# nktoan/h-edit

Measured on AMD Instinct MI355X. Metric: edited images/sec (512^2, 50 steps, K Langevin), higher is better.
Workload: dtype bf16

## Files before the change

### h-edit_amd/csrc/c_api.hip

```cpp
#include "../../include/hedit.h"
#include <exception>
#include <map>
#include <mutex>
#include <new>
#include <set>
#include <utility>

#include "common.h"
#include "kernels.h"

static thread_local std::string g_last_error;
void hedit_set_error(const std::string& msg) { g_last_error = msg; }

int hedit_abi_catch() noexcept {
  try {
    try {
      throw;
    } catch (const std::bad_alloc&) {
      g_last_error = "out of host memory inside libhedit_hip";
    } catch (const std::exception& e) {
      g_last_error = std::string("C++ exception inside libhedit_hip: ") + e.what();
    } catch (...) {
      g_last_error = "unknown C++ exception inside libhedit_hip";
    }
// ... 133 lines not shown
int hedit_k_gemm_plan_splits(int M, int N, int K, int chunk_kt) { return gemm_plan_splits(M, N, K, chunk_kt); }

int hedit_k_gemm(const void* A, const void* W, const float* bias, const void* residual, void* C, int M, int N,
                 int K, int lda, int ldc, int ldr, int mode, int Hin, int Win, int Cin, int Hout, int Wout,
                 int splits, void* partial_ws, void* stream) try {
  ARG_CHECK(A && W && C, "gemm args");
  GemmParams p{};
  p.A = reinterpret_cast<const bf16_t*>(A);
  p.W = reinterpret_cast<const bf16_t*>(W);
  p.M = M; p.N = N; p.K = K; p.lda = lda; p.mode = mode;
  p.Hin = Hin; p.Win = Win; p.Cin = Cin; p.Hout = Hout; p.Wout = Wout;
  p.bias = bias;
  p.residual = reinterpret_cast<const bf16_t*>(residual);
  p.ldr = ldr;
  p.C = reinterpret_cast<bf16_t*>(C);
  p.ldc = ldc;
  if (splits < 0) {
    const int kt = K / 64;
    const int s = gemm_pick_splits(M, N, K, -splits);
    p.chunk_kt = (kt + s - 1) / s;
    return gemm_launch(p, 1, nullptr, S(stream));
  }
  const int s = gemm_pick_splits(M, N, K, splits);
  return gemm_launch(p, s, reinterpret_cast<float*>(partial_ws), S(stream));
} catch (...) { return hedit_abi_catch(); }

int hedit_k_conv_gn(const void* A, const void* W, const float* bias, const void* residual, void* C, int M, int N, int K, int ldc,
                    int ldr, int mode, int Hin, int Win, int Cin, int Hout, int Wout, int splits, void* partial_ws, float* gn_part,
                    void* stream) try {
  ARG_CHECK(A && W && C && gn_part, "conv_gn args");
  GemmParams p{};
  p.A = reinterpret_cast<const bf16_t*>(A);
  p.W = reinterpret_cast<const bf16_t*>(W);
  p.M = M; p.N = N; p.K = K; p.lda = Cin; p.mode = mode;
  p.Hin = Hin; p.Win = Win; p.Cin = Cin; p.Hout = Hout; p.Wout = Wout;
  p.bias = bias;
  p.residual = reinterpret_cast<const bf16_t*>(residual);
  p.ldr = ldr;
  p.C = reinterpret_cast<bf16_t*>(C);
  p.ldc = ldc;
  p.gn_part = gn_part;
  if (splits < 0) {
    const int kt = K / 64;
    const int s = gemm_pick_splits(M, N, K, -splits);
    p.chunk_kt = (kt + s - 1) / s;
    return gemm_launch(p, 1, nullptr, S(stream));
  }
  const int s = gemm_pick_splits(M, N, K, splits);
  return gemm_launch(p, s, reinterpret_cast<float*>(partial_ws), S(stream));
} catch (...) { return hedit_abi_catch(); }

int hedit_k_groupnorm_from_parts(const void* x, void* y, const float* gamma, const float* beta, int B, int HW, int C, int G,
                                 float eps, int silu, const float* part_a, int ca, const float* part_b, int cb, void* ws,
                                 void* stream) try {
  ARG_CHECK(x && y && gamma && beta && part_a && ws, "groupnorm_from_parts args");
  return groupnorm_from_parts_launch(reinterpret_cast<const bf16_t*>(x), reinterpret_cast<bf16_t*>(y), gamma, beta, B, HW, C, G,
                                     eps, silu, part_a, ca, part_b, cb, reinterpret_cast<float*>(ws), S(stream));
} catch (...) { return hedit_abi_catch(); }

int hedit_k_pack_geglu(const float* w, const float* bias, void* w_packed_bf16, float* bias_packed, int inner, int K,
                       void* stream) try {
  ARG_CHECK(w && w_packed_bf16, "pack_geglu args");
  int rc = pack_geglu_rows_launch(w, reinterpret_cast<bf16_t*>(w_packed_bf16), nullptr, 2 * inner, K, S(stream));
  if (rc != HEDIT_OK || !bias) return rc;
  ARG_CHECK(bias_packed, "pack_geglu: bias_packed");
  return pack_geglu_rows_launch(bias, nullptr, bias_packed, 2 * inner, 1, S(stream));
} catch (...) { return hedit_abi_catch(); }

int hedit_k_gemm_geglu(const void* A, const void* w_packed, const float* bias_packed, void* C, int M, int inner, int K,
                       int lda, int ldc, void* stream) try {
  ARG_CHECK(A && w_packed && C, "gemm_geglu args");
  GemmParams p{};
  p.A = reinterpret_cast<const bf16_t*>(A);
  p.W = reinterpret_cast<const bf16_t*>(w_packed);
  p.M = M; p.N = 2 * inner; p.K = K; p.lda = lda; p.mode = 0;
  p.bias = bias_packed;
  p.C = reinterpret_cast<bf16_t*>(C);
  p.ldc = ldc;
  p.geglu = 1;
  return gemm_launch(p, 1, nullptr, S(stream));
} catch (...) { return hedit_abi_catch(); }

int hedit_k_ffn_channels(void) { return ffn_fused_channels(); }
size_t hedit_k_ffn_stream_bytes(int with_outer_layers) { return ffn_stream_bytes(with_outer_layers, with_outer_layers); }
size_t hedit_k_ffn_bias_bytes(void) { return ffn_bias_bytes(); }

int hedit_k_ffn_pack(const float* w1, const float* b1, const float* w2, const float* w_pre, const float* w_post, void* stream_out,
                     float* bias1_out, void* stream) try {
  ARG_CHECK(w1 && b1 && w2 && stream_out && bias1_out && ((w_pre == nullptr) == (w_post == nullptr)), "ffn_pack args");
  const int outer = w_pre != nullptr;
  bf16_t* so = reinterpret_cast<bf16_t*>(stream_out);
  int rc = ffn_pack_launch(w1, 1, outer, outer, so, S(stream));
  if (rc == HEDIT_OK) rc = ffn_pack_launch(w2, 2, outer, outer, so, S(stream));
  if (rc == HEDIT_OK && outer) rc = ffn_pack_launch(w_pre, 0, 1, 1, so, S(stream));
  if (rc == HEDIT_OK && outer) rc = ffn_pack_launch(w_post, 3, 1, 1, so, S(stream));
  if (rc != HEDIT_OK) return rc;
  return ffn_pack_bias_launch(b1, bias1_out, S(stream));
} catch (...) { return hedit_abi_catch(); }

int hedit_k_ffn_fused(const void* x, int64_t ldx, const float* gamma, const float* beta, float eps, const void* w_stream,
                      const float* bias1_packed, const float* bias2, void* out, int64_t ldo, int M, int C, void* stream) try {
  FfnParams f{};
  f.x = reinterpret_cast<const bf16_t*>(x); f.ldx = (long)ldx; f.gamma = gamma; f.beta = beta; f.eps = eps;
  f.stream = reinterpret_cast<const bf16_t*>(w_stream); f.bias1p = bias1_packed; f.bias2 = bias2;
  f.out = reinterpret_cast<bf16_t*>(out); f.ldo = (long)ldo; f.M = M; f.C = C;
  return ffn_fused_launch(f, S(stream));
} catch (...) { return hedit_abi_catch(); }

int hedit_k_ffn_chain(const void* a, int64_t lda, const void* t1, int64_t ldt1, const void* x, int64_t ldx, const float* bias_pre,
                      const float* gamma, const float* beta, float eps, const void* w_stream, const float* bias1_packed, const float* bias2,
                      const float* bias_post, void* out, int64_t ldo, int M, int C, void* stream) try {
  ARG_CHECK(a && t1 && x, "ffn_chain args");
  FfnParams f{};
  f.a = reinterpret_cast<const bf16_t*>(a); f.lda = (long)lda;
  f.x = reinterpret_cast<const bf16_t*>(t1); f.ldx = (long)ldt1;
  f.r2 = reinterpret_cast<const bf16_t*>(x); f.ldr2 = (long)ldx;
  f.bias_pre = bias_pre; f.bias_post = bias_post;
  f.gamma = gamma; f.beta = beta; f.eps = eps;
  f.stream = reinterpret_cast<const bf16_t*>(w_stream); f.bias1p = bias1_packed; f.bias2 = bias2;
  f.out = reinterpret_cast<bf16_t*>(out); f.ldo = (long)ldo; f.M = M; f.C = C;
  return ffn_fused_launch(f, S(stream));
} catch (...) { return hedit_abi_catch(); }

size_t hedit_k_lin_chain_stream_bytes(int n_out) { return lin_chain_stream_bytes(n_out == 3 ? 4 : 2); }

int hedit_k_lin_chain_pack(const float* w_pre, const float* w0, const float* w1, const float* w2, float scale0, void* stream_out,
                           void* stream) try {
  ARG_CHECK(w_pre && w0 && stream_out && ((w1 == nullptr) == (w2 == nullptr)), "lin_chain_pack args");
  const int layers = w1 ? 4 : 2;
  bf16_t* so = reinterpret_cast<bf16_t*>(stream_out);
  int rc = lin_chain_pack_launch(w_pre, 0, 1.f, layers, so, S(stream));
  if (rc == HEDIT_OK) rc = lin_chain_pack_launch(w0, 1, scale0, layers, so, S(stream));
  if (rc == HEDIT_OK && w1) rc = lin_chain_pack_launch(w1, 2, 1.f, layers, so, S(stream));
  if (rc == HEDIT_OK && w1) rc = lin_chain_pack_launch(w2, 3, 1.f, layers, so, S(stream));
  return rc;
} catch (...) { return hedit_abi_catch(); }

int hedit_k_lin_chain(const void* a, int64_t lda, const void* r1, int64_t ldr1, const float* gn_ss, int rows_per_image,
                      const float* bias_pre, const float* gamma, const float* beta, float eps, const void* w_stream, void* out_mid,
                      int64_t ldmid, void* out_q, int64_t ldq, void* out_k, int64_t ldk, void* out, int64_t ldo, int M, int C,
                      void* stream) try {
  LinChainParams c{};
  c.a = reinterpret_cast<const bf16_t*>(a); c.lda = (long)lda; c.r1 = reinterpret_cast<const bf16_t*>(r1); c.ldr1 = (long)ldr1;
  c.bias_pre = bias_pre; c.gamma = gamma; c.beta = beta; c.eps = eps; c.stream = reinterpret_cast<const bf16_t*>(w_stream);
  c.out_mid = reinterpret_cast<bf16_t*>(out_mid); c.ldmid = (long)ldmid; c.out = reinterpret_cast<bf16_t*>(out); c.ldo = (long)ldo;
  c.M = M; c.C = C; c.gn_ss = gn_ss; c.rows_per_image = rows_per_image;
  c.out_q = reinterpret_cast<bf16_t*>(out_q); c.ldq = (long)ldq; c.out_k = reinterpret_cast<bf16_t*>(out_k); c.ldk = (long)ldk;
  return lin_chain_launch(c, S(stream));
} catch (...) { return hedit_abi_catch(); }

int hedit_storage_is_f16(void) { return HEDIT_F16; }

int hedit_test_set_flags(int flags) try {
  ARG_CHECK(flags >= 0 && flags <= 15, "hedit_test_set_flags: bit 0 drained ring waits, bit 1 exact self-attention pass, bit 2 pixel-UNet GroupNorm statistics path flipped, bit 3 no persistent linear kernel");
  g_test_flags.store(flags, std::memory_order_relaxed);
  return HEDIT_OK;
} catch (...) { return hedit_abi_catch(); }

int hedit_k_lin_chain_sched(const void* a, int64_t lda, const void* r1, int64_t ldr1, const float* gn_ss, int rows_per_image,
                            const float* bias_pre, const float* gamma, const float* beta, float eps, const void* w_stream, void* out_mid,
                            int64_t ldmid, void* out_q, int64_t ldq, void* out_k, int64_t ldk, void* out, int64_t ldo, int M, int C,
                            int sched, void* stream) try {
  LinChainParams c{};
  c.a = reinterpret_cast<const bf16_t*>(a); c.lda = (long)lda; c.r1 = reinterpret_cast<const bf16_t*>(r1); c.ldr1 = (long)ldr1;
  c.bias_pre = bias_pre; c.gamma = gamma; c.beta = beta; c.eps = eps; c.stream = reinterpret_cast<const bf16_t*>(w_stream);
  c.out_mid = reinterpret_cast<bf16_t*>(out_mid); c.ldmid = (long)ldmid; c.out = reinterpret_cast<bf16_t*>(out); c.ldo = (long)ldo;
  c.M = M; c.C = C; c.gn_ss = gn_ss; c.rows_per_image = rows_per_image;
  c.out_q = reinterpret_cast<bf16_t*>(out_q); c.ldq = (long)ldq; c.out_k = reinterpret_cast<bf16_t*>(out_k); c.ldk = (long)ldk;
  return lin_chain_launch_sched(c, sched, S(stream));
} catch (...) { return hedit_abi_catch(); }

size_t hedit_k_groupnorm_ws_bytes(int B, int HW, int C) { return groupnorm_ws_bytes(B, HW, C); }

int hedit_k_groupnorm_affine(const void* x, const float* gamma, const float* beta, int B, int HW, int C, int G, float eps, void* ws,
                             float* ss_out, void* stream) try {
  ARG_CHECK(x && gamma && beta && ws && ss_out, "groupnorm_affine args");
  const float* ss = nullptr;
  int rc = groupnorm_affine_launch(reinterpret_cast<const bf16_t*>(x), gamma, beta, B, HW, C, G, eps, reinterpret_cast<float*>(ws), S(stream), &ss);
  if (rc != HEDIT_OK) return rc;
  HIP_TRY(hipMemcpyAsync(ss_out, ss, (size_t)B * C * 2 * sizeof(float), hipMemcpyDeviceToDevice, S(stream)));
  return HEDIT_OK;
} catch (...) { return hedit_abi_catch(); }

int hedit_k_groupnorm(const void* x, void* y, const float* gamma, const float* beta, int B, int HW, int C, int G,
                      float eps, int silu, void* ws, void* stream) try {
  ARG_CHECK(x && y && gamma && beta && ws, "groupnorm args");
  return groupnorm_launch(reinterpret_cast<const bf16_t*>(x), reinterpret_cast<bf16_t*>(y), gamma, beta, B, HW, C, G,
                          eps, silu, reinterpret_cast<float*>(ws), S(stream));
} catch (...) { return hedit_abi_catch(); }

int hedit_k_layernorm(const void* x, void* y, const float* gamma, const float* beta, int64_t rows, int C, float eps,
                      void* stream) try {
  ARG_CHECK(x && y && gamma && beta, "layernorm args");
  return layernorm_launch(reinterpret_cast<const bf16_t*>(x), reinterpret_cast<bf16_t*>(y), gamma, beta, (long)rows, C, eps, S(stream));
} catch (...) { return hedit_abi_catch(); }

int hedit_k_geglu(const void* x, void* y, int64_t rows, int inner, void* stream) try {
  ARG_CHECK(x && y, "geglu args");
  return geglu_launch(reinterpret_cast<const bf16_t*>(x), reinterpret_cast<bf16_t*>(y), (long)rows, inner, S(stream));
} catch (...) { return hedit_abi_catch(); }

int hedit_k_self_attn(const void* q, int ldq, const void* k, int ldk, const void* vt, int64_t ldvt, void* out, int ldo,
                      int B, int N, int heads, int d, const int32_t* qk_src, const int32_t* kv_src, void* stream) try {
  ARG_CHECK(q && k && vt && out, "self_attn args");
  SelfAttnParams p{};
  p.q = reinterpret_cast<const bf16_t*>(q); p.ldq = ldq;
  p.k = reinterpret_cast<const bf16_t*>(k); p.ldk = ldk;
  p.vt = reinterpret_cast<const bf16_t*>(vt); p.ldvt = (long)ldvt;
  p.out = reinterpret_cast<bf16_t*>(out); p.ldo = ldo;
  p.B = B; p.N = N; p.heads = heads; p.d = d; p.qk_src = qk_src; p.kv_src = kv_src;
  return self_attn_launch(p, S(stream));
} catch (...) { return hedit_abi_catch(); }

int hedit_k_cross_attn(const void* q, int ldq, const void* k, int ldk, const void* vt, int64_t ldvt, void* out, int ldo,
                       int B, int N, int heads, int d, const hedit_p2p_plan* plan, float* store, void* stream) try {
  ARG_CHECK(q && k && vt && out && plan, "cross_attn args");
  CrossAttnParams p{};
  p.q = reinterpret_cast<const bf16_t*>(q); p.ldq = ldq;
  p.k = reinterpret_cast<const bf16_t*>(k); p.ldk = ldk;
  p.vt = reinterpret_cast<const bf16_t*>(vt); p.ldvt = (long)ldvt;
  p.out = reinterpret_cast<bf16_t*>(out); p.ldo = ldo;
  p.B = B; p.N = N; p.heads = heads; p.d = d;
  p.n_pairs = plan->n_pairs; p.pair_src = plan->pair_src; p.pair_tar = plan->pair_tar;
  p.mixT = reinterpret_cast<const bf16_t*>(plan->mixT); p.bvec = plan->bvec;
  p.singles = plan->singles; p.n_single = plan->n_single;
  p.store = store;
  return cross_attn_launch(p, S(stream));
} catch (...) { return hedit_abi_catch(); }

int hedit_k_attn_probs(const void* q, int ldq, const void* k, int ldk, float* probs, int B, int N, int M, int kstride,
                       int heads, int d, void* stream) try {
  ARG_CHECK(q && k && probs, "attn_probs args");
  AttnProbsParams p{};
  p.q = reinterpret_cast<const bf16_t*>(q); p.ldq = ldq;
  p.k = reinterpret_cast<const bf16_t*>(k); p.ldk = ldk;
  p.probs = probs; p.B = B; p.N = N; p.M = M; p.kstride = kstride; p.heads = heads; p.d = d;
  return attn_probs_launch(p, S(stream));
} catch (...) { return hedit_abi_catch(); }

int hedit_k_attn_apply(const float* probs, const void* vt, int64_t ldvt, void* out, int ldo, int B, int N, int M,
                       int kstride, int heads, int d, void* stream) try {
  ARG_CHECK(probs && vt && out, "attn_apply args");
  AttnProbsParams p{};
  p.probs = const_cast<float*>(probs);
  p.vt = reinterpret_cast<const bf16_t*>(vt); p.ldvt = (long)ldvt;
  p.out = reinterpret_cast<bf16_t*>(out); p.ldo = ldo;
  p.B = B; p.N = N; p.M = M; p.kstride = kstride; p.heads = heads; p.d = d;
  return attn_apply_launch(p, S(stream));
} catch (...) { return hedit_abi_catch(); }

int hedit_k_pack_conv3x3(const float* w, void* out, int O, int I, void* stream) try {
  ARG_CHECK(w && out, "pack args");
  return pack_conv3x3_launch(w, reinterpret_cast<bf16_t*>(out), O, I, S(stream));
} catch (...) { return hedit_abi_catch(); }

int hedit_k_f32_to_bf16(const float* x, void* y, int64_t n, void* stream) try {
  ARG_CHECK(x && y, "cast args");
  return f32_to_bf16_launch(x, reinterpret_cast<bf16_t*>(y), (long)n, S(stream));
} catch (...) { return hedit_abi_catch(); }

int hedit_k_groupnorm_stats(const void* x, void* y, const float* gamma, const float* beta, int B, int HW, int C, int G,
                            float eps, int silu, void* ws, float* stats, void* stream) try {
  ARG_CHECK(x && y && gamma && beta && ws && stats, "groupnorm_stats args");
  return groupnorm_launch(reinterpret_cast<const bf16_t*>(x), reinterpret_cast<bf16_t*>(y), gamma, beta, B, HW, C, G,
                          eps, silu, reinterpret_cast<float*>(ws), S(stream), stats);
} catch (...) { return hedit_abi_catch(); }

size_t hedit_k_groupnorm_bwd_ws_bytes(int B, int HW, int C) { return groupnorm_bwd_ws_bytes(B, HW, C); }

int hedit_k_groupnorm_bwd(const void* x, const void* dy, const void* add, void* dx, const float* gamma, const float* beta,
                          const float* stats, int B, int HW, int C, int G, int silu, void* ws, void* stream) try {
  ARG_CHECK(x && dy && dx && gamma && beta && stats && ws, "groupnorm_bwd args");
  return groupnorm_bwd_launch(reinterpret_cast<const bf16_t*>(x), reinterpret_cast<const bf16_t*>(dy),
                              reinterpret_cast<const bf16_t*>(add), reinterpret_cast<bf16_t*>(dx), gamma, beta, stats, B, HW, C,
                              G, silu, reinterpret_cast<float*>(ws), S(stream));
} catch (...) { return hedit_abi_catch(); }

int hedit_k_softmax_rows(const float* s, void* p, int64_t rows, int N, float scale, void* stream) try {
  ARG_CHECK(s && p, "softmax_rows args");
  return softmax_rows_launch(s, reinterpret_cast<bf16_t*>(p), (long)rows, N, scale, S(stream));
} catch (...) { return hedit_abi_catch(); }

int hedit_k_softmax_blockdiag(const float* s, void* p, int64_t rows, int T, int ld, float scale, void* stream) try {
  ARG_CHECK(s && p, "softmax_blockdiag args");
  return softmax_blockdiag_launch(s, reinterpret_cast<bf16_t*>(p), (long)rows, T, ld, scale, S(stream));
} catch (...) { return hedit_abi_catch(); }

int hedit_k_softmax_bwd(const void* p, const float* dp, void* ds, int64_t rows, int N, float scale, void* stream) try {
  ARG_CHECK(p && dp && ds, "softmax_bwd args");
  return softmax_bwd_launch(reinterpret_cast<const bf16_t*>(p), dp, reinterpret_cast<bf16_t*>(ds), (long)rows, N, scale, S(stream));
} catch (...) { return hedit_abi_catch(); }

int hedit_k_transpose(const void* src, void* dst, int R, int C, void* stream) try {
  ARG_CHECK(src && dst, "transpose args");
  return transpose_bf16_launch(reinterpret_cast<const bf16_t*>(src), reinterpret_cast<bf16_t*>(dst), R, C, S(stream));
} catch (...) { return hedit_abi_catch(); }

int hedit_k_sum2x2(const void* du, void* dx, int B, int H, int W, int C, void* stream) try {
  ARG_CHECK(du && dx, "sum2x2 args");
  return sum2x2_launch(reinterpret_cast<const bf16_t*>(du), reinterpret_cast<bf16_t*>(dx), B, H, W, C, S(stream));
} catch (...) { return hedit_abi_catch(); }

int hedit_k_pack_conv3x3_dgrad(const float* w, void* out, int O, int I, void* stream) try {
  ARG_CHECK(w && out, "pack args");
  return pack_conv3x3_dgrad_launch(w, reinterpret_cast<bf16_t*>(out), O, I, S(stream));
} catch (...) { return hedit_abi_catch(); }

// ... 110 lines not shown
```

### h-edit_amd/csrc/norm.hip

```cpp
#include <stdlib.h>
#include "common.h"
#include "kernels.h"

namespace {


constexpr int GN_MAXV = 2;

__global__ __launch_bounds__(256) void gn_partial_kernel(const bf16_t* __restrict__ x, float* __restrict__ part,
                                                         int HW, int C, int G, int nslab) {
  extern __shared__ float lds[];
  const int CV = C / 8;
  const int slab = blockIdx.x, b = blockIdx.y;
  const int pix_per = (HW + nslab - 1) / nslab;
  const int p0 = slab * pix_per;
  int p1 = p0 + pix_per;
  if (p1 > HW) p1 = HW;
  const int R = CV <= 256 ? 256 / CV : 1;
  const int r = CV <= 256 ? threadIdx.x / CV : 0;
  const int cv0 = CV <= 256 ? threadIdx.x % CV : threadIdx.x;
  const bool active = r < R;
  float s[GN_MAXV][8], q[GN_MAXV][8];
#pragma unroll
  for (int v = 0; v < GN_MAXV; ++v)
// ... 450 lines not shown
  }
  acc = wave_sum(acc);
  if (lane == 0) out[n] = acc + (b0 ? b0[n] : 0.f) + (b1 ? b1[n] : 0.f);
}

__global__ void timestep_embed_kernel(float t, float* out, int dim) {
  const int half = dim / 2;
  for (int i = threadIdx.x; i < half; i += blockDim.x) {
    const float fr = expf(-9.210340371976184f * (float)i / (float)half);
    const float a = t * fr;
    out[i] = cosf(a);
    out[half + i] = sinf(a);
  }
}

__global__ void timestep_embed_ddpm_kernel(float t, float* out, int dim) {
  const int half = dim / 2;
  for (int i = threadIdx.x; i < half; i += blockDim.x) {
    const float fr = expf(-9.210340371976184f / (float)(half - 1) * (float)i);
    const float a = t * fr;
    out[i] = sinf(a);
    out[half + i] = cosf(a);
  }
  if ((dim & 1) && threadIdx.x == 0) out[dim - 1] = 0.f;
}

constexpr int CI_PIX = 128;
__global__ __launch_bounds__(256) void conv_in_kernel(const float* __restrict__ x, const float* __restrict__ w, const float* __restrict__ bias,
                                                      bf16_t* __restrict__ y, int B, int Cin, int H, int Wd, int Cout) {
  extern __shared__ float lds[];
  const int K = Cin * 9;
  float* sw = lds;
  float* sx = lds + (long)K * Cout;
  for (int i = threadIdx.x; i < K * Cout; i += 256) {
    const int co = i / K, k = i - co * K;
    sw[k * Cout + co] = w[i];
  }
  const long pix0 = (long)blockIdx.x * CI_PIX;
  const long npix = (long)B * H * Wd;
  for (int i = threadIdx.x; i < CI_PIX * K; i += 256) {
    const int k = i / CI_PIX, pl = i - k * CI_PIX;
    const long pix = pix0 + pl;
    float v = 0.f;
    if (pix < npix) {
      const int ox = (int)(pix % Wd), oy = (int)((pix / Wd) % H), b = (int)(pix / ((long)Wd * H));
      const int ci = k / 9, tap = k - ci * 9;
      const int iy = oy + tap / 3 - 1, ix = ox + tap % 3 - 1;
      if ((unsigned)iy < (unsigned)H && (unsigned)ix < (unsigned)Wd) v = x[(((long)b * Cin + ci) * H + iy) * Wd + ix];
    }
    sx[k * CI_PIX + pl] = v;
  }
  __syncthreads();
  const int CV = Cout / 8;
  for (int i = threadIdx.x; i < (CI_PIX / 4) * CV; i += 256) {
    const int pg = i / CV, cv = i - pg * CV;
    float acc[4][8];
#pragma unroll
    for (int q = 0; q < 4; ++q)
#pragma unroll
      for (int j = 0; j < 8; ++j) acc[q][j] = bias[cv * 8 + j];
    for (int k = 0; k < K; ++k) {
      const float4 xv = *reinterpret_cast<const float4*>(sx + k * CI_PIX + pg * 4);
      const float4 w0 = *reinterpret_cast<const float4*>(sw + k * Cout + cv * 8);
      const float4 w1 = *reinterpret_cast<const float4*>(sw + k * Cout + cv * 8 + 4);
      const float xq[4] = {xv.x, xv.y, xv.z, xv.w};
#pragma unroll
      for (int q = 0; q < 4; ++q) {
        acc[q][0] += xq[q] * w0.x; acc[q][1] += xq[q] * w0.y; acc[q][2] += xq[q] * w0.z; acc[q][3] += xq[q] * w0.w;
        acc[q][4] += xq[q] * w1.x; acc[q][5] += xq[q] * w1.y; acc[q][6] += xq[q] * w1.z; acc[q][7] += xq[q] * w1.w;
      }
    }
#pragma unroll
    for (int q = 0; q < 4; ++q) {
      const long pix = pix0 + pg * 4 + q;
      if (pix < npix) *reinterpret_cast<uint4*>(y + pix * Cout + cv * 8) = pack8(acc[q]);
    }
  }
}

__global__ __launch_bounds__(256) void conv_out_kernel(const bf16_t* __restrict__ x, const bf16_t* __restrict__ w, const float* __restrict__ bias,
                                                       float* __restrict__ y, int B, int H, int Wd, int C, int Cout) {
  const int lane = threadIdx.x & 63;
  const long pix = (long)blockIdx.x * 4 + (threadIdx.x >> 6);
  if (pix >= (long)B * H * Wd) return;
  const int ox = (int)(pix % Wd);
  const int oy = (int)((pix / Wd) % H);
  const int b = (int)(pix / ((long)Wd * H));
  const int CV = C / 8;
  float acc[4] = {0.f, 0.f, 0.f, 0.f};
  for (int idx = lane; idx < 9 * CV; idx += 64) {
    const int tap = idx / CV, cv = idx - tap * CV;
    const int iy = oy + tap / 3 - 1, ix = ox + tap % 3 - 1;
    if ((unsigned)iy >= (unsigned)H || (unsigned)ix >= (unsigned)Wd) continue;
    uint4 u = *reinterpret_cast<const uint4*>(x + (((long)b * H + iy) * Wd + ix) * C + cv * 8);
    float f[8];
    unpack8(u, f);
    for (int co = 0; co < Cout; ++co) {
      uint4 uw = *reinterpret_cast<const uint4*>(w + ((long)co * 9 + tap) * C + cv * 8);
      float ww[8];
      unpack8(uw, ww);
#pragma unroll
      for (int j = 0; j < 8; ++j) acc[co] += f[j] * ww[j];
    }
  }
  for (int co = 0; co < Cout; ++co) {
    float v = wave_sum(acc[co]);
    if (lane == 0) y[(((long)b * Cout + co) * H + oy) * Wd + ox] = v + bias[co];
  }
}

__global__ __launch_bounds__(256) void gn_small_kernel(const bf16_t* __restrict__ x, bf16_t* __restrict__ y,
                                                       const float* __restrict__ gamma, const float* __restrict__ beta,
                                                       int HW, int C, int G, float eps, int silu, float* __restrict__ stats) {
  extern __shared__ uint32_t gs_pairs[];
  __shared__ float red[8];
  const int g = blockIdx.x, b = blockIdx.y, tid = threadIdx.x;
  const int cpg = C / G, ppp = cpg / 2;
  const int npair = HW * ppp;
  const uint32_t* xin = reinterpret_cast<const uint32_t*>(x + (long)b * HW * C + g * cpg);
  float s = 0.f, q = 0.f;
  for (int i = tid; i < npair; i += 256) {
    const int pix = i / ppp, j = i - pix * ppp;
    const uint32_t u = xin[(long)pix * (C / 2) + j];
    gs_pairs[i] = u;
    const float a = st_lo(u), c = st_hi(u);
    s += a; s += c;
    q += a * a; q += c * c;
  }
  s = wave_sum(s);
  q = wave_sum(q);
  if ((tid & 63) == 0) { red[(tid >> 6) * 2] = s; red[(tid >> 6) * 2 + 1] = q; }
  __syncthreads();
  s = ((red[0] + red[2]) + red[4]) + red[6];
  q = ((red[1] + red[3]) + red[5]) + red[7];
  const float n = (float)HW * (float)cpg;
  const float m = s / n;
  float var = q / n - m * m;
  var = var < 0.f ? 0.f : var;
  const float rstd = rsqrtf(var + eps);
  if (stats && tid == 0) *reinterpret_cast<float2*>(stats + ((long)b * G + g) * 2) = make_float2(m, rstd);
  uint32_t* yout = reinterpret_cast<uint32_t*>(y + (long)b * HW * C + g * cpg);
  for (int i = tid; i < npair; i += 256) {
    const int pix = i / ppp, j = i - pix * ppp;
    const uint32_t u = gs_pairs[i];
    const int c0 = g * cpg + 2 * j;
    const float sc0 = rstd * gamma[c0], sc1 = rstd * gamma[c0 + 1];
    float a = st_lo(u) * sc0 + (beta[c0] - m * sc0);
    float c = st_hi(u) * sc1 + (beta[c0 + 1] - m * sc1);
    if (silu) { a = silu_f(a); c = silu_f(c); }
    yout[(long)pix * (C / 2) + j] = pack_bf16x2(a, c);
  }
}

__global__ __launch_bounds__(256) void gn_fold_kernel(const float* __restrict__ pa, int npa, const float* __restrict__ pb, int npb,
                                                      float* __restrict__ out, int units, int ppg) {
  __shared__ float red[8];
  const int g = blockIdx.x, b = blockIdx.y, tid = threadIdx.x;
  const int total = units * ppg;
  float s = 0.f, q = 0.f;
  for (int e = tid; e < total; e += 256) {
    const int u = e / ppg, j = e - u * ppg;
    const int pr = g * ppg + j;
    const long row = (long)b * units + u;
    const float2 v = pr < npa ? *reinterpret_cast<const float2*>(pa + (row * npa + pr) * 2)
                              : *reinterpret_cast<const float2*>(pb + (row * npb + (pr - npa)) * 2);
    s += v.x;
    q += v.y;
  }
  s = wave_sum(s);
  q = wave_sum(q);
  if ((tid & 63) == 0) { red[(tid >> 6) * 2] = s; red[(tid >> 6) * 2 + 1] = q; }
  __syncthreads();
  if (tid == 0) {
    s = ((red[0] + red[2]) + red[4]) + red[6];
    q = ((red[1] + red[3]) + red[5]) + red[7];
    *reinterpret_cast<float2*>(out + ((long)b * gridDim.x + g) * 2) = make_float2(s, q);
  }
}

int gn_nslab(int B, int HW, int C) {
  (void)B;
  const int CV = C / 8;
  const int R = CV <= 256 ? 256 / CV : 1;
  int n = HW / (R * 8);
  int cap = HW / 256;
  cap = cap < 32 ? 32 : (cap > 64 ? 64 : cap);
  if (HW >= 512 * 512) cap = 128;
  if (n > cap) n = cap;
  if (n < 1) n = 1;
  return n;
}

}

size_t groupnorm_ws_bytes(int B, int HW, int C) {
  const int nslab = gn_nslab(B, HW, C);
  return ((size_t)B * nslab * 64 * 2 + (size_t)B * C * 2) * sizeof(float);
}

int groupnorm_launch(const bf16_t* x, bf16_t* y, const float* gamma, const float* beta, int B, int HW,
                     int C, int G, float eps, int silu, float* ws, hipStream_t st, float* stats) {
  ARG_CHECK(C % 8 == 0 && C % G == 0 && G <= 64, "groupnorm: C % 8, C % G, G <= 64");
  ARG_CHECK(C / 8 <= 256 * GN_MAXV, "groupnorm: C too large");
  if (HW < 1024 && (C / G) % 2 == 0 && (size_t)HW * (C / G) * 2 <= 60 * 1024) {
    hipLaunchKernelGGL(gn_small_kernel, dim3(G, B), dim3(256), (size_t)HW * (C / G) * 2, st, x, y, gamma, beta, HW, C, G, eps, silu, stats);
    LAUNCH_CHECK();
    return HEDIT_OK;
  }
  const int nslab = gn_nslab(B, HW, C);
  float* part = ws;
  float* ss = ws + (size_t)B * nslab * 64 * 2;
  const int CV = C / 8;
  const int R = CV <= 256 ? 256 / CV : 1;
  const size_t lds = (size_t)R * C * 2 * sizeof(float);
  ARG_CHECK(lds <= 64 * 1024, "groupnorm: LDS");
  hipLaunchKernelGGL(gn_partial_kernel, dim3(nslab, B), dim3(256), lds, st, x, part, HW, C, G, nslab);
  LAUNCH_CHECK();
  const long total_v = (long)B * HW * CV;
  const bool rows_form = CV <= 256 && HW >= 1024;
  if (!rows_form || stats) {
    hipLaunchKernelGGL(gn_finalize_kernel, dim3(B), dim3(256), 0, st, part, gamma, beta, ss, HW, C, G, nslab, eps, stats);
    LAUNCH_CHECK();
  }
  if (rows_form) {
    int ns = (int)(4096 / (B > 0 ? B : 1)) + 1;
    const int max_ns = HW / (R * 8) > 0 ? HW / (R * 8) : 1;
    if (ns > max_ns) ns = max_ns;
    {
      int pix = HW / ns / (4 * R) * (4 * R);
      if (pix < 4 * R) pix = 4 * R;
      ns = (HW + pix - 1) / pix;
    }
    hipLaunchKernelGGL(gn_apply_rows_kernel, dim3(ns, B), dim3(256), 0, st, x, y, part, gamma, beta, HW, C, G, nslab, eps, silu, ns);
    LAUNCH_CHECK();
    return HEDIT_OK;
  }
  hipLaunchKernelGGL(gn_apply_kernel, dim3(ew_grid(total_v)), dim3(256), 0, st, x, y, ss, total_v, HW, C, silu);
  LAUNCH_CHECK();
  return HEDIT_OK;
}

bool groupnorm_from_parts_supported(int HW, int C, int G) {
  return HW >= 1024 && HW % 128 == 0 && C % 8 == 0 && C / 8 <= 256 && C % G == 0 && (C / G) % 2 == 0 && G <= 64;
}
size_t groupnorm_from_parts_ws_bytes(int B) { return (size_t)B * 64 * 2 * sizeof(float); }

int groupnorm_from_parts_launch(const bf16_t* x, bf16_t* y, const float* gamma, const float* beta, int B, int HW, int C, int G,
                                float eps, int silu, const float* part_a, int ca, const float* part_b, int cb, float* ws,
                                hipStream_t st) {
  ARG_CHECK(groupnorm_from_parts_supported(HW, C, G), "groupnorm_from_parts: shape");
  ARG_CHECK(part_a && ca > 0 && ca % 2 == 0 && cb >= 0 && cb % 2 == 0 && ca + cb == C && (cb == 0) == (part_b == nullptr),
            "groupnorm_from_parts: the pair statistics must cover the C channels");
  hipLaunchKernelGGL(gn_fold_kernel, dim3(G, B), dim3(256), 0, st, part_a, ca / 2, part_b, cb / 2, ws, HW / 128, C / G / 2);
  LAUNCH_CHECK();
  const int CV = C / 8, R = 256 / CV;
  int ns = (int)(4096 / (B > 0 ? B : 1)) + 1;
  const int max_ns = HW / (R * 8) > 0 ? HW / (R * 8) : 1;
  if (ns > max_ns) ns = max_ns;
  int pix = HW / ns / (4 * R) * (4 * R);
  if (pix < 4 * R) pix = 4 * R;
  ns = (HW + pix - 1) / pix;
  hipLaunchKernelGGL(gn_apply_rows_kernel, dim3(ns, B), dim3(256), 0, st, x, y, ws, gamma, beta, HW, C, G, 1, eps, silu, ns);
  LAUNCH_CHECK();
  return HEDIT_OK;
}

int groupnorm_affine_launch(const bf16_t* x, const float* gamma, const float* beta, int B, int HW, int C, int G, float eps,
                            float* ws, hipStream_t st, const float** ss_out) {
  ARG_CHECK(C % 8 == 0 && C % G == 0 && G <= 64, "groupnorm: C % 8, C % G, G <= 64");
  ARG_CHECK(C / 8 <= 256 * GN_MAXV, "groupnorm: C too large");
  const int nslab = gn_nslab(B, HW, C);
  float* part = ws;
  float* ss = ws + (size_t)B * nslab * 64 * 2;
  const int CV = C / 8;
  const int R = CV <= 256 ? 256 / CV : 1;
  const size_t lds = (size_t)R * C * 2 * sizeof(float);
  ARG_CHECK(lds <= 64 * 1024, "groupnorm: LDS");
  hipLaunchKernelGGL(gn_partial_kernel, dim3(nslab, B), dim3(256), lds, st, x, part, HW, C, G, nslab);
  LAUNCH_CHECK();
  hipLaunchKernelGGL(gn_finalize_kernel, dim3(B), dim3(256), 0, st, part, gamma, beta, ss, HW, C, G, nslab, eps, (float*)nullptr);
  LAUNCH_CHECK();
  *ss_out = ss;
  return HEDIT_OK;
}

static int ln_narrow_lanes(int C) {
  if (C % 64 == 0 && C / 64 <= LNN_MAXV) return 8;
  if (C % 128 == 0 && C / 128 <= LNN_MAXV) return 16;
  if (C % 256 == 0 && C / 256 <= LNN_MAXV) return 32;
  return 0;
}

bool splitk_reduce_ln_supported(int C) { return C % 8 == 0 && ln_narrow_lanes(C) != 0; }

int splitk_reduce_ln_launch(const float* partial, int splits, const float* bias, const bf16_t* residual, int ldr, bf16_t* out,
                            bf16_t* y, const float* gamma, const float* beta, long rows, int C, float eps, hipStream_t st) {
  const int lanes = ln_narrow_lanes(C);
  ARG_CHECK(lanes != 0 && splits >= 1, "splitk_reduce_ln: unsupported row width");
  const LnReduce rd{partial, splits, bias, residual, ldr};
  if (lanes == 8) hipLaunchKernelGGL((layernorm_narrow_kernel<8, true>), dim3(cdiv(rows, 32)), dim3(256), 0, st, out, y, gamma, beta, rows, C, eps, rd);
  else if (lanes == 16) hipLaunchKernelGGL((layernorm_narrow_kernel<16, true>), dim3(cdiv(rows, 16)), dim3(256), 0, st, out, y, gamma, beta, rows, C, eps, rd);
  else hipLaunchKernelGGL((layernorm_narrow_kernel<32, true>), dim3(cdiv(rows, 8)), dim3(256), 0, st, out, y, gamma, beta, rows, C, eps, rd);
  LAUNCH_CHECK();
  return HEDIT_OK;
}

int layernorm_launch(const bf16_t* x, bf16_t* y, const float* gamma, const float* beta, long rows, int C,
                     float eps, hipStream_t st) {
  ARG_CHECK(C % 8 == 0 && C / 8 <= 64 * LN_MAXV, "layernorm: C");
  const LnReduce none{};
  bf16_t* xx = const_cast<bf16_t*>(x);
  switch (ln_narrow_lanes(C)) {
    case 8:
      hipLaunchKernelGGL((layernorm_narrow_kernel<8, false>), dim3(cdiv(rows, 32)), dim3(256), 0, st, xx, y, gamma, beta, rows, C, eps, none);
      LAUNCH_CHECK();
      return HEDIT_OK;
    case 16:
      hipLaunchKernelGGL((layernorm_narrow_kernel<16, false>), dim3(cdiv(rows, 16)), dim3(256), 0, st, xx, y, gamma, beta, rows, C, eps, none);
      LAUNCH_CHECK();
      return HEDIT_OK;
    case 32:
      hipLaunchKernelGGL((layernorm_narrow_kernel<32, false>), dim3(cdiv(rows, 8)), dim3(256), 0, st, xx, y, gamma, beta, rows, C, eps, none);
      LAUNCH_CHECK();
      return HEDIT_OK;
    default: break;
  }
  hipLaunchKernelGGL(layernorm_kernel, dim3(cdiv(rows, 4)), dim3(256), 0, st, x, y, gamma, beta, rows, C, eps);
  LAUNCH_CHECK();
  return HEDIT_OK;
}

int geglu_launch(const bf16_t* x, bf16_t* y, long rows, int inner, hipStream_t st) {
  ARG_CHECK(inner % 8 == 0, "geglu: inner % 8");
  hipLaunchKernelGGL(geglu_kernel, dim3(ew_grid(rows * (inner / 8))), dim3(256), 0, st, x, y, rows, inner);
  LAUNCH_CHECK();
  return HEDIT_OK;
}

int concat_launch(const bf16_t* a, int ca, const bf16_t* b, int cb, bf16_t* y, long rows, hipStream_t st, const RowMap* b_map,
                  int rows_per_image) {
  ARG_CHECK(ca % 8 == 0 && cb % 8 == 0, "concat: channels % 8");
  if (b_map) {
    ARG_CHECK(rows_per_image > 0 && rows % rows_per_image == 0 && rows / rows_per_image <= HEDIT_ROWMAP_MAX, "concat: row map");
    hipLaunchKernelGGL(concat_mapped_kernel, dim3(ew_grid(rows * (((a ? ca : 0) + cb) / 8))), dim3(256), 0, st, a, ca, b, cb, y, rows,
                       rows_per_image, *b_map);
    LAUNCH_CHECK();
    return HEDIT_OK;
  }
  if (a == nullptr) {
    hipLaunchKernelGGL(concat_right_kernel, dim3(ew_grid(rows * (cb / 8))), dim3(256), 0, st, b, ca, cb, y, rows);
    LAUNCH_CHECK();
    return HEDIT_OK;
  }
  hipLaunchKernelGGL(concat_kernel, dim3(ew_grid(rows * ((ca + cb) / 8))), dim3(256), 0, st, a, ca, b, cb, y, rows);
  LAUNCH_CHECK();
  return HEDIT_OK;
}
// ... 242 lines not shown
```

Baseline: 2.635.

## Add wide small-image GroupNorm kernel with 16-byte loads over multiple groups per block

Adds a GroupNorm kernel for small spatial sizes in which each block handles R adjacent groups. This lets each pixel's channel run be loaded and stored as 16-byte vectors, with many loads kept in flight before being staged in LDS. Per-channel scale and shift are precomputed into a shared table, and blocks are swizzled across the grid. It targets the latent-UNet GroupNorms, whose old one-group-per-block kernel used 4-byte pair accesses. It falls back to the old kernel on misaligned pointers or a test flag, at the cost of more LDS per block and fewer groups per grid.

Result: no change. 2.652 (median of 6 runs) (+0.7%).

```diff
diff --git a/h-edit_amd/csrc/c_api.hip b/h-edit_amd/csrc/c_api.hip
--- a/h-edit_amd/csrc/c_api.hip
+++ b/h-edit_amd/csrc/c_api.hip
@@ -309,7 +309,7 @@
 int hedit_storage_is_f16(void) { return HEDIT_F16; }
 
 int hedit_test_set_flags(int flags) try {
-  ARG_CHECK(flags >= 0 && flags <= 15, "hedit_test_set_flags: bit 0 drained ring waits, bit 1 exact self-attention pass, bit 2 pixel-UNet GroupNorm statistics path flipped, bit 3 no persistent linear kernel");
+  ARG_CHECK(flags >= 0 && flags <= 31, "hedit_test_set_flags: bit 0 drained ring waits, bit 1 exact self-attention pass, bit 2 pixel-UNet GroupNorm statistics path flipped, bit 3 no persistent linear kernel, bit 4 one-group-per-block small-image GroupNorm");
   g_test_flags.store(flags, std::memory_order_relaxed);
   return HEDIT_OK;
 } catch (...) { return hedit_abi_catch(); }
diff --git a/h-edit_amd/csrc/norm.hip b/h-edit_amd/csrc/norm.hip
--- a/h-edit_amd/csrc/norm.hip
+++ b/h-edit_amd/csrc/norm.hip
@@ -626,6 +626,113 @@
   }
 }
 
+constexpr int GW_MAXR = 8;
+constexpr int GW_MAXC = 320;
+constexpr int GW_INFLIGHT = 10;
+
+__global__ __launch_bounds__(256) void gn_wide_kernel(const bf16_t* __restrict__ x, bf16_t* __restrict__ y,
+                                                      const float* __restrict__ gamma, const float* __restrict__ beta,
+                                                      int HW, int C, int G, int R, float eps, int silu, float* __restrict__ stats) {
+  extern __shared__ __attribute__((aligned(16))) uint32_t gw_pairs[];
+  __shared__ float red[GW_MAXR * 8];
+  __shared__ float2 mr[GW_MAXR];
+  __shared__ __attribute__((aligned(16))) float2 tab[GW_MAXC];
+  int run = blockIdx.x;
+  if (gridDim.x % 8 == 0) run = (run & 7) * (gridDim.x >> 3) + (run >> 3);
+  const int g0 = run * R, b = blockIdx.y, tid = threadIdx.x;
+  const int cpg = C / G, ppp = cpg / 2;
+  const int rp = R * ppp;
+  const int rv = rp / 4;
+  const int npiece = HW * rv;
+  uint4* lds4 = reinterpret_cast<uint4*>(gw_pairs);
+  const bf16_t* xin = x + (long)b * HW * C + g0 * cpg;
+  const int dq = 256 / rv, dr = 256 - dq * rv;
+  {
+    int pix = tid / rv, c = tid - pix * rv;
+    for (int i0 = tid; i0 < npiece; i0 += 256 * GW_INFLIGHT) {
+      uint4 v[GW_INFLIGHT];
+#pragma unroll
+      for (int k = 0; k < GW_INFLIGHT; ++k) {
+        v[k] = *reinterpret_cast<const uint4*>(xin + (long)(pix < HW ? pix : HW - 1) * C + c * 8);
+        pix += dq; c += dr;
+        if (c >= rv) { c -= rv; ++pix; }
+      }
+#pragma unroll
+      for (int k = 0; k < GW_INFLIGHT; ++k)
+        asm volatile("" : "+v"(v[k].x), "+v"(v[k].y), "+v"(v[k].z), "+v"(v[k].w));
+#pragma unroll
+      for (int k = 0; k < GW_INFLIGHT; ++k) {
+        const int i = i0 + k * 256;
+        if (i < npiece) lds4[i] = v[k];
+      }
+    }
+  }
+  __syncthreads();
+  const int npair = HW * ppp;
+  for (int gi = 0; gi < R; ++gi) {
+    float s = 0.f, q = 0.f;
+    for (int i = tid; i < npair; i += 256) {
+      int at = i;
+      if (R > 1) { const int pix = i / ppp; at = pix * rp + gi * ppp + (i - pix * ppp); }
+      const uint32_t u = gw_pairs[at];
+      const float a = st_lo(u), c = st_hi(u);
+      s += a; s += c;
+      q += a * a; q += c * c;
+    }
+    s = wave_sum(s);
+    q = wave_sum(q);
+    if ((tid & 63) == 0) { red[gi * 8 + (tid >> 6) * 2] = s; red[gi * 8 + (tid >> 6) * 2 + 1] = q; }
+  }
+  __syncthreads();
+  if (tid < R) {
+    const float* rd = red + tid * 8;
+    const float s = ((rd[0] + rd[2]) + rd[4]) + rd[6];
+    const float q = ((rd[1] + rd[3]) + rd[5]) + rd[7];
+    const float n = (float)HW * (float)cpg;
+    const float m = s / n;
+    float var = q / n - m * m;
+    var = var < 0.f ? 0.f : var;
+    const float rstd = rsqrtf(var + eps);
+    mr[tid] = make_float2(m, rstd);
+    if (stats) *reinterpret_cast<float2*>(stats + ((long)b * G + g0 + tid) * 2) = make_float2(m, rstd);
+  }
+  __syncthreads();
+  for (int cl = tid; cl < R * cpg; cl += 256) {
+    const float2 st = mr[cl / cpg];
+    const int c0 = g0 * cpg + cl;
+    const float sc = st.y * gamma[c0];
+    tab[cl] = make_float2(sc, beta[c0] - st.x * sc);
+  }
+  __syncthreads();
+  bf16_t* yout = y + (long)b * HW * C + g0 * cpg;
+  int pix = tid / rv, c = tid - pix * rv;
+  for (int i = tid; i < npiece; i += 256) {
+    const uint4 u4 = lds4[i];
+    const uint32_t u[4] = {u4.x, u4.y, u4.z, u4.w};
+    uint32_t o[4];
+#pragma unroll
+    for (int k = 0; k < 4; ++k) {
+      const float4 t = *reinterpret_cast<const float4*>(tab + c * 8 + 2 * k);
+      float a = st_lo(u[k]) * t.x + t.y;
+      float e = st_hi(u[k]) * t.z + t.w;
+      if (silu) { a = silu_f(a); e = silu_f(e); }
+      o[k] = pack_bf16x2(a, e);
+    }
+    *reinterpret_cast<uint4*>(yout + (long)pix * C + c * 8) = make_uint4(o[0], o[1], o[2], o[3]);
+    pix += dq; c += dr;
+    if (c >= rv) { c -= rv; ++pix; }
+  }
+}
+
+int gn_wide_run(int HW, int C, int G) {
+  const int cpg = C / G;
+  const size_t group_bytes = (size_t)HW * cpg * 2;
+  int R = 1;
+  while ((R * cpg * 2) % 16 != 0 && G % (2 * R) == 0 && 2 * R <= GW_MAXR && 2 * R * group_bytes <= 60 * 1024) R *= 2;
+  if ((R * cpg * 2) % 16 != 0 || R * cpg > GW_MAXC || G % R != 0) return 0;
+  return R;
+}
+
 __global__ __launch_bounds__(256) void gn_fold_kernel(const float* __restrict__ pa, int npa, const float* __restrict__ pb, int npb,
                                                       float* __restrict__ out, int units, int ppg) {
   __shared__ float red[8];
@@ -677,6 +784,13 @@
   ARG_CHECK(C % 8 == 0 && C % G == 0 && G <= 64, "groupnorm: C % 8, C % G, G <= 64");
   ARG_CHECK(C / 8 <= 256 * GN_MAXV, "groupnorm: C too large");
   if (HW < 1024 && (C / G) % 2 == 0 && (size_t)HW * (C / G) * 2 <= 60 * 1024) {
+    const int R = gn_wide_run(HW, C, G);
+    if (R > 0 && !(hedit_test_flags() & 16) && (reinterpret_cast<uintptr_t>(x) | reinterpret_cast<uintptr_t>(y)) % 16 == 0) {
+      hipLaunchKernelGGL(gn_wide_kernel, dim3(G / R, B), dim3(256), (size_t)R * HW * (C / G) * 2, st, x, y, gamma, beta, HW, C, G, R, eps,
+                         silu, stats);
+      LAUNCH_CHECK();
+      return HEDIT_OK;
+    }
     hipLaunchKernelGGL(gn_small_kernel, dim3(G, B), dim3(256), (size_t)HW * (C / G) * 2, st, x, y, gamma, beta, HW, C, G, eps, silu, stats);
     LAUNCH_CHECK();
     return HEDIT_OK;
```
